# urbste/MultiCol-SLAM

Measured on AMD Instinct MI355X. Metric: Mfeatures/s extract+match, 3-cam 754x480 multi-frame, higher is better.
Workload: dtype u8+i32 (images, Hamming) / f64 (omni model)

## Files before the change

### include/mcs_c.h

```cpp
#ifndef MCS_C_H
#define MCS_C_H
#include <stdint.h>
#include <stddef.h>
#ifdef __cplusplus
extern "C" {
#endif

#define MCS_OK 0
#define MCS_ERR_INVALID (-1)
#define MCS_ERR_HIP (-2)
#define MCS_ERR_CAPACITY (-3)
#define MCS_ERR_UNSUPPORTED (-4)

#define MCS_ABI_VERSION 10

#define MCS_MAX_POLY 16
#define MCS_MAX_LEVELS 16

typedef struct mcs_ctx mcs_ctx;
typedef struct mcs_extractor mcs_extractor;

typedef struct { float x, y, size, angle, response; int32_t octave, class_id; } mcs_keypoint;

typedef struct {
// ... 43 lines not shown
int mcs_extractor_patch_ties(mcs_extractor*, int back, int* listed, int* recomputed);
int mcs_describe_fast_bound(const mcs_ocam* cam, int desc_size, double* bound);
int mcs_selftest_describe_fast(mcs_ctx*, const mcs_ocam* cam, uint64_t seed, int n, double* max_abs_diff);
int mcs_describe_fast_table(const mcs_ocam* cam, double* table, int* rows, int* row_len, int* e0, int* bins_per_octave, double* info6);
int mcs_describe_fast_table_packed(const mcs_ocam* cam, void* packed, int* row_bytes, double* f32_term);

int mcs_extract_batch_strided(mcs_extractor*, int nimg, const uint8_t* images, size_t image_pitch, int image_stride, const uint8_t* masks,
                              size_t mask_pitch, int mask_stride, const mcs_ocam* cams, int32_t* nkp, mcs_keypoint* keypoints, uint8_t* desc,
                              uint8_t* descmask, double* rays, size_t out_image_pitch_rows, int out_row_stride);

int mcs_extractor_status(mcs_extractor*);

int mcs_extractor_tap_level(mcs_extractor*, int img, int level, int blurred, uint8_t* out );
int mcs_extractor_tap_candidates(mcs_extractor*, int img, int level, uint32_t* out , int cap, int* n);
int mcs_extractor_tap_selected(mcs_extractor*, int img, int level, uint32_t* out, int cap, int* n);

typedef struct {
	const uint8_t* desc; const uint8_t* mask; const uint8_t* valid; const int32_t* group; int32_t n; int32_t stride;
	int32_t block_rows; int64_t block_pitch_rows;
} mcs_desc_set;
int mcs_match_topk(mcs_ctx*, const mcs_desc_set* q, const mcs_desc_set* t, int dim, int K, int count_thresh, mcs_mem_kind kind,
                   int32_t* out_dist, int32_t* out_idx, int32_t* out_count_le);

int mcs_match_topk_batched(mcs_ctx*, int nsets, const mcs_desc_set* q, size_t q_set_pitch_rows, const mcs_desc_set* t,
                           size_t t_set_pitch_rows, int dim, int K, int count_thresh, mcs_mem_kind kind, int32_t* out_dist,
                           int32_t* out_idx, int32_t* out_count_le);

int mcs_search_kf_kf(mcs_ctx*, int nsets, const mcs_desc_set* kf1, size_t pitch1_rows, const mcs_desc_set* kf2, size_t pitch2_rows, int dim,
                     double nnratio, int K, mcs_mem_kind kind, int32_t* match12, int32_t* nmatches, int32_t* fallbacks );
int mcs_search_kf_f(mcs_ctx*, int nsets, const mcs_desc_set* kf, size_t pitchKF_rows, const mcs_desc_set* frame, size_t pitchF_rows, int dim,
// ... 156 lines not shown
```

### multicol-slam_amd/__init__.py

```python
import ctypes as C

import numpy as np

from . import _capi
from ._capi import (KP_DTYPE, MASKS_RESIDENT, MEM_DEVICE, MEM_HOST, DescSet, ExtractorParams, McsError, Ocam, check, lib, make_ocam, np_ptr)

__all__ = ["Context", "Extractor", "McsError", "KP_DTYPE", "make_ocam", "ExtractorParams", "MEM_HOST", "MEM_DEVICE"]


class Context:

    def __init__(self, device=0, stream=None):
        self.h = C.c_void_p()
        check(lib().mcs_ctx_create(device, C.c_void_p(stream) if stream else None, C.byref(self.h)))
        self.device = device

    def close(self):
        if getattr(self, "h", None):
            lib().mcs_ctx_destroy(self.h)
            self.h = None

    def __del__(self):
        try:
            self.close()
# ... 185 lines not shown
        check(lib().mcs_extractor_tap_level(self.h, img, level, int(blurred), np_ptr(out)))
        return out

    def _tap(self, fn, img, level):
        buf = np.zeros(1 << 17, np.uint32)
        n = C.c_int32()
        check(fn(self.h, img, level, np_ptr(buf), len(buf), C.byref(n)))
        rec = buf[:n.value]
        return (rec & 0xFFF).astype(np.int32), ((rec >> 12) & 0xFFF).astype(np.int32), (rec >> 24).astype(np.int32)

    def tap_candidates(self, img, level):
        return self._tap(lib().mcs_extractor_tap_candidates, img, level)

    def tap_selected(self, img, level):
        return self._tap(lib().mcs_extractor_tap_selected, img, level)
```

### multicol-slam_amd/_capi.py

```python
import ctypes as C
import os

import numpy as np

_HERE = os.path.dirname(os.path.abspath(__file__))
LIB_PATH = os.environ.get("MCS_HIP_LIB", os.path.join(_HERE, "libmcs_hip.so"))

MCS_OK, MCS_ERR_INVALID, MCS_ERR_HIP, MCS_ERR_CAPACITY, MCS_ERR_UNSUPPORTED = 0, -1, -2, -3, -4
MEM_HOST, MEM_DEVICE = 0, 1
MASKS_RESIDENT = C.c_void_p(1)
MAX_POLY = 16


class McsError(RuntimeError):
    def __init__(self, code, msg):
        super().__init__("libmcs_hip error %d: %s" % (code, msg))
        self.code = code


class KeyPoint(C.Structure):
    _fields_ = [("x", C.c_float), ("y", C.c_float), ("size", C.c_float), ("angle", C.c_float), ("response", C.c_float),
                ("octave", C.c_int32), ("class_id", C.c_int32)]


# ... 23 lines not shown
    o = Ocam()
    o.c, o.d, o.e, o.u0, o.v0 = cam["c"], cam["d"], cam["e"], cam["u0"], cam["v0"]
    for i, v in enumerate(cam["p"]):
        o.p[i] = v
    o.p_deg = len(cam["p"])
    for i, v in enumerate(cam["invP"]):
        o.invP[i] = v
    o.invP_deg = len(cam["invP"])
    o.width, o.height = cam["width"], cam["height"]
    return o


EXPORTS = [
    "mcs_last_error", "mcs_abi_version", "mcs_device_count", "mcs_ctx_create", "mcs_ctx_destroy", "mcs_ctx_synchronize", "mcs_extractor_create",
    "mcs_extractor_destroy", "mcs_extractor_set_masks", "mcs_extractor_kp_capacity", "mcs_extractor_levels", "mcs_extract_batch", "mcs_extractor_status",
    "mcs_extractor_tap_level", "mcs_extractor_tap_candidates", "mcs_extractor_tap_selected", "mcs_match_topk",
    "mcs_match_topk_batched", "mcs_descriptor_distance", "mcs_descriptor_distance_masked", "mcs_ctx_enable_timing",
    "mcs_ctx_kernel_ms", "mcs_ctx_join", "mcs_ctx_set_async_search", "mcs_ctx_search_fence", "mcs_search_kf_kf", "mcs_search_kf_f", "mcs_search_triangulation", "mcs_search_kf_f_sweep",
    "mcs_search_triangulation_sweep", "mcs_search_kf_kf_ring", "mcs_rows_valid", "mcs_extractor_set_describe", "mcs_extractor_describe_stats", "mcs_extractor_tie_stats", "mcs_extractor_set_tie_band", "mcs_extractor_fix_ties", "mcs_extractor_tie_counts", "mcs_extractor_set_tie_capture", "mcs_extractor_patch_ties", "mcs_describe_fast_bound",
    "mcs_selftest_describe_fast", "mcs_describe_fast_table", "mcs_describe_fast_table_packed", "mcs_extract_batch_strided", "mcs_rig_pack_headers", "mcs_rig_rows_valid",
    "mcs_search_by_projection", "mcs_window_match", "mcs_window_best", "mcs_rotation_consistency", "mcs_world_to_cam", "mcs_distinctive_descriptors", "mcs_selftest_shared_reciprocal", "mcs_vocabulary_create", "mcs_vocabulary_destroy", "mcs_bow_transform", "mcs_copy_narrow", "mcs_ctx_result_stream", "mcs_ctx_stream_conflicts", "mcs_ctx_transfer_stream", "mcs_host_alloc", "mcs_host_free",
    "mcs_vocabulary_set_words", "mcs_bow_vector", "mcs_kfdb_create", "mcs_kfdb_destroy", "mcs_kfdb_clear", "mcs_kfdb_size", "mcs_kfdb_add", "mcs_kfdb_erase",
    "mcs_kfdb_set_covisibility", "mcs_kfdb_detect_relocalisation", "mcs_kfdb_detect_loop", "mcs_kfdb_score",
    "mcs_sim3_create", "mcs_sim3_destroy", "mcs_sim3_set_ransac_parameters", "mcs_sim3_iterate", "mcs_sim3_best", "mcs_sim3_info",
    "mcs_sim3_hypotheses", "mcs_sim3_draw",
    "mcs_triangulate_matches", "mcs_create_new_map_points",
    "mcs_frustum", "mcs_search_local_points",
]

WINDOW_RATIO, WINDOW_BEST, WINDOW_INITIALIZE = 1, 2, 3

# ... 85 lines not shown
    L.mcs_extractor_fix_ties.argtypes = [vp, C.POINTER(C.c_int)]
    L.mcs_extractor_set_tie_capture.argtypes = [vp, C.c_int, C.c_int]
    L.mcs_extractor_patch_ties.argtypes = [vp, C.c_int, C.POINTER(C.c_int), C.POINTER(C.c_int)]
    L.mcs_extractor_tie_counts.argtypes = [vp, C.POINTER(C.c_uint64), C.POINTER(C.c_uint64), C.POINTER(C.c_double)]
    L.mcs_describe_fast_bound.argtypes = [C.POINTER(Ocam), C.c_int, C.POINTER(C.c_double)]
    L.mcs_selftest_describe_fast.argtypes = [vp, C.POINTER(Ocam), C.c_uint64, C.c_int, C.POINTER(C.c_double)]
    L.mcs_describe_fast_table.argtypes = [C.POINTER(Ocam), vp, C.POINTER(C.c_int), C.POINTER(C.c_int), C.POINTER(C.c_int), C.POINTER(C.c_int), vp]
    L.mcs_describe_fast_table_packed.argtypes = [C.POINTER(Ocam), vp, C.POINTER(C.c_int), C.POINTER(C.c_double)]
    L.mcs_extract_batch.argtypes = [vp, C.c_int, vp, C.c_size_t, C.c_int, vp, C.c_size_t, C.c_int, vp, C.c_int, vp, vp, vp, vp, vp]
    L.mcs_extract_batch_strided.argtypes = [vp, C.c_int, vp, C.c_size_t, C.c_int, vp, C.c_size_t, C.c_int, vp, vp, vp, vp, vp, vp, C.c_size_t, C.c_int]
    L.mcs_rig_pack_headers.argtypes = [vp, vp, C.c_int, C.c_int, vp, C.c_int]
    L.mcs_rig_rows_valid.argtypes = [vp, vp, C.c_int, C.c_int, C.c_int, vp, vp]
    L.mcs_extractor_tap_level.argtypes = [vp, C.c_int, C.c_int, C.c_int, vp]
    L.mcs_extractor_tap_candidates.argtypes = [vp, C.c_int, C.c_int, vp, C.c_int, i32p]
    L.mcs_extractor_tap_selected.argtypes = [vp, C.c_int, C.c_int, vp, C.c_int, i32p]
    L.mcs_match_topk.argtypes = [vp, C.POINTER(DescSet), C.POINTER(DescSet), C.c_int, C.c_int, C.c_int, C.c_int, vp, vp, vp]
    L.mcs_match_topk_batched.argtypes = [vp, C.c_int, C.POINTER(DescSet), C.c_size_t, C.POINTER(DescSet), C.c_size_t, C.c_int,
                                         C.c_int, C.c_int, C.c_int, vp, vp, vp]
    srch = [vp, C.c_int, C.POINTER(DescSet), C.c_size_t, C.POINTER(DescSet), C.c_size_t, C.c_int, C.c_double, C.c_int, C.c_int, vp, vp, vp]
    L.mcs_search_kf_kf.argtypes = srch
    L.mcs_search_kf_f.argtypes = srch
    L.mcs_search_triangulation.argtypes = [vp, C.c_int, C.POINTER(DescSet), C.c_size_t, C.POINTER(DescSet), C.c_size_t, vp, vp, vp, C.c_int,
                                           C.c_int, C.c_int, C.c_int, vp, vp, vp]
    L.mcs_search_kf_kf_ring.argtypes = [vp, C.c_int, C.c_int, C.c_int, C.POINTER(DescSet), C.c_size_t, C.c_int, C.c_double, C.c_int, C.c_int, vp, vp, vp]
    L.mcs_search_kf_f_sweep.argtypes = [vp, C.c_int, C.POINTER(DescSet), C.c_size_t, C.c_int, C.POINTER(DescSet), C.c_size_t, C.c_int, C.c_double, C.c_int,
                                        C.c_int, vp, vp, vp]
    L.mcs_search_triangulation_sweep.argtypes = [vp, C.c_int, C.POINTER(DescSet), C.c_size_t, C.POINTER(DescSet), C.c_size_t, vp, vp, vp, C.c_size_t,
                                                 C.c_int, C.c_int, C.c_int, C.c_int, vp, vp, vp]
    L.mcs_rows_valid.argtypes = [vp, vp, C.c_int, C.c_int, vp]
    L.mcs_search_by_projection.argtypes = [vp, C.POINTER(ProjectionSet), C.POINTER(FrameView), C.c_double, C.c_double, C.c_int, C.c_int, vp, vp]
# ... 54 lines not shown
```

### multicol-slam_amd/csrc/mcs_capi.hip

```cpp
#include "mcs_common.h"

#include <algorithm>
#include <cmath>
#include <cstdio>
#include <cstdlib>
#include <cstring>
#include <map>
#include <string>
#include <vector>

namespace mcs {
bool upload_describe_tables(const signed char* pattern);
void launch_single_distance(const uint8_t* a, const uint8_t* b, const uint8_t* ma, const uint8_t* mb, int dim, int* out, hipStream_t s);
void describe_host(int mode, int descSize, const signed char* pattern, const OcamDev* cam, int undistort, int level, float levelScale, int row, int col, float angle,
                   const HostLevel& L, uint8_t* desc, uint8_t* mask);
void launch_tie_capture(const ExtractBuffers& b, const PyrDesc& hd, int nimg, int maxTies, uint8_t* devOut, hipStream_t s);
void launch_selftest_fast_model(const OcamDev* cam, const double* tab, unsigned long long seed, int n, int width, int height, unsigned long long* maxDiff, hipStream_t s);
static const signed char kPattern[2048] = {
#include "learned_pattern_64_orb.inc"
};
}

using namespace mcs;

// ... 192 lines not shown
	int* d_fbCount = nullptr; uint32_t *d_fbList = nullptr, *d_preList = nullptr; unsigned long long* d_fbStats = nullptr; unsigned long long* d_tieMin = nullptr; void* d_aux = nullptr;
	int describeMode = 0; double guardEps = kDefaultGuardEps;
	uint32_t* d_tieList = nullptr; double tieBand = 0.0; unsigned long long tieFixed = 0;
	struct TieSlot { uint8_t* host = nullptr; uint8_t* dev = nullptr; hipEvent_t ev = nullptr; ExtractBuffers b{}; int nimg = 0; std::vector<OcamDev> cams; long long seq = -1; bool patched = false; };
	std::vector<TieSlot> tieRing; int tieMax = 0; long long batchSeq = 0; hipStream_t patchStream = nullptr; uint8_t* h_patchRows = nullptr;
	unsigned long long tieWindowMisses = 0;
	TieSlot hostTie;
	struct CamFast { OcamDev key; GTabInfo info; std::vector<double> tab; };
	std::vector<CamFast> camCache;
	double* d_gTab = nullptr;
	DevBuf inImg, inMask;
	int* d_nkp = nullptr; mcs_keypoint* d_kps = nullptr; uint8_t *d_odesc = nullptr, *d_omask = nullptr; double* d_rays = nullptr;
	ExtractBuffers last{};
	int lastN = 0;
	uint8_t* d_resMask = nullptr; int resMaskN = 0;
	int* h_status = nullptr;
	struct Graph { ExtractBuffers key; int nimg; hipGraphExec_t exec; };
	std::vector<Graph> graphs;
	long graphHits = 0, graphMisses = 0;
};

extern "C" {

const char* mcs_last_error(void) { return mcs_err().c_str(); }
int mcs_abi_version(void) { return MCS_ABI_VERSION; }

int mcs_device_count(int* n) {
	if (!n) return fail(MCS_ERR_INVALID, "null");
	HIPCHK(hipGetDeviceCount(n));
	return MCS_OK;
// ... 281 lines not shown
	for (int v = -kHalfPatch; v <= kHalfPatch; ++v)
		for (int u = -umax[std::abs(v)]; u <= umax[std::abs(v)]; ++u) { disc.push_back((signed char)u); disc.push_back((signed char)v); }
	if (disc.size() != 845 * 2) { delete e; return fail(MCS_ERR_INVALID, "internal: disc size"); }
	for (int v = 0; v <= kHalfPatch; ++v) hd.umax[v] = umax[v];
	if (!upload_describe_tables(kPattern)) { delete e; return fail(MCS_ERR_HIP, "pattern tables: upload failed (or the distinct-point rounds of mcs_describe.hip do not fit this pattern)"); }

	hd.chainFits = 0; hd.chainRegOff = 0;
	if (getenv("MCS_PYR_CHAIN") && !taps.empty()) {
		std::vector<int> table;
		if (pyramid_chain_table(hd, taps.data(), &table)) {
			hd.chainFits = 1; hd.chainRegOff = (int)taps.size();
			taps.resize(taps.size() + (table.size() * sizeof(int) + sizeof(ResizeTap) - 1) / sizeof(ResizeTap));
			memcpy(taps.data() + hd.chainRegOff, table.data(), table.size() * sizeof(int));
		}
	}
	const size_t B = max_batch;
#define ALLOC(ptr, bytes) do { hipError_t _e = hipMalloc((void**)&(ptr), (bytes)); if (_e != hipSuccess) { mcs_extractor_destroy(e); return fail(MCS_ERR_HIP, std::string("hipMalloc ") + #ptr + ": " + hipGetErrorString(_e)); } } while (0)
	ALLOC(e->d_desc, sizeof(PyrDesc));
	ALLOC(e->d_cells, sizeof(CellInfo) * e->cells.size());
	ALLOC(e->d_taps, sizeof(ResizeTap) * std::max<size_t>(taps.size(), 1));
	ALLOC(e->d_maskMap, sizeof(short) * maps.size());
	ALLOC(e->d_pyr, B * hd.pyrBytes);
	ALLOC(e->d_blur, B * hd.pyrBytes);
	ALLOC(e->d_slots, B * hd.slotsPerImage * sizeof(uint32_t));
	ALLOC(e->d_dense, B * hd.densePerImage * sizeof(uint32_t));
	ALLOC(e->d_knode, B * hd.densePerImage * sizeof(unsigned short));
	ALLOC(e->d_sel, B * hd.selPerImage * sizeof(uint32_t));
	ALLOC(e->d_selAngle, B * hd.selPerImage * sizeof(float));
	ALLOC(e->d_cellCount, B * hd.cellsPerImage * sizeof(int));
	ALLOC(e->d_denseCount, B * nl * sizeof(int));
	ALLOC(e->d_selCount, B * nl * sizeof(int));
	ALLOC(e->d_status, sizeof(int));
	ALLOC(e->d_cams, B * sizeof(OcamDev));
	const size_t slotsPerImage = (size_t)(hd.kpCap + kSlotAlign - 1) / kSlotAlign * kSlotAlign;
	ALLOC(e->d_fbCount, 3 * sizeof(int));
	if (hipHostMalloc((void**)&e->h_status, 2 * sizeof(int), hipHostMallocDefault) != hipSuccess) { (void)hipGetLastError(); e->h_status = nullptr; }
	ALLOC(e->d_tieList, B * slotsPerImage * sizeof(uint32_t));
	ALLOC(e->d_fbList, B * slotsPerImage * sizeof(uint32_t));
	ALLOC(e->d_preList, B * slotsPerImage * sizeof(uint32_t));
	ALLOC(e->d_fbStats, 2 * sizeof(unsigned long long));
	ALLOC(e->d_tieMin, sizeof(unsigned long long));
	ALLOC(e->d_aux, B * slotsPerImage * describe_aux_bytes());
	ALLOC(e->d_gTab, B * (size_t)kGDevDoubles * sizeof(double));
	ALLOC(e->d_nkp, B * sizeof(int));
	ALLOC(e->d_kps, B * hd.kpCap * sizeof(mcs_keypoint));
	ALLOC(e->d_odesc, B * hd.kpCap * (size_t)hd.descSize);
	ALLOC(e->d_omask, B * hd.kpCap * (size_t)hd.descSize);
	ALLOC(e->d_rays, B * hd.kpCap * 3 * sizeof(double));
#undef ALLOC
	HIPCHK(hipMemcpy(e->d_desc, &hd, sizeof(PyrDesc), hipMemcpyHostToDevice));
	HIPCHK(hipMemcpy(e->d_cells, e->cells.data(), sizeof(CellInfo) * e->cells.size(), hipMemcpyHostToDevice));
	if (!taps.empty()) HIPCHK(hipMemcpy(e->d_taps, taps.data(), sizeof(ResizeTap) * taps.size(), hipMemcpyHostToDevice));
	HIPCHK(hipMemcpy(e->d_maskMap, maps.data(), sizeof(short) * maps.size(), hipMemcpyHostToDevice));
	HIPCHK(hipMemset(e->d_status, 0, sizeof(int)));
	HIPCHK(hipMemset(e->d_fbCount, 0, 3 * sizeof(int)));
	HIPCHK(hipMemset(e->d_fbStats, 0, 2 * sizeof(unsigned long long)));
	{ const unsigned long long inf = 0x7FF0000000000000ull; HIPCHK(hipMemcpy(e->d_tieMin, &inf, sizeof(inf), hipMemcpyHostToDevice)); }
	if (hipHostMalloc((void**)&e->hostTie.host, sizeof(TieCaptureHeader) + (size_t)kHostTieSlots * sizeof(TieCaptureEntry), hipHostMallocDefault) == hipSuccess) {
		memset(e->hostTie.host, 0, sizeof(TieCaptureHeader));
		e->hostTie.dev = (uint8_t*)device_view(e->hostTie.host);
	} else { (void)hipGetLastError(); e->hostTie.host = nullptr; }
	if (getenv("MCS_DESCRIBE_EXACT")) e->describeMode = 1;
	HIPCHK(hipMemset(e->d_pyr, 0, B * hd.pyrBytes));
	HIPCHK(hipMemset(e->d_blur, 0, B * hd.pyrBytes));
	ctx->extractors.push_back(e);
	*out = e;
// ... 5 lines not shown
	e->tieRing.clear(); e->tieMax = 0;
	if (e->h_patchRows) { (void)hipHostFree(e->h_patchRows); e->h_patchRows = nullptr; }
	if (e->patchStream) { (void)hipStreamSynchronize(e->patchStream); (void)hipStreamDestroy(e->patchStream); e->patchStream = nullptr; }
}

int mcs_extractor_destroy(mcs_extractor* e) {
	if (!e) return MCS_OK;
	(void)hipSetDevice(e->ctx->device);
	(void)hipStreamSynchronize(e->ctx->stream);
	{
		std::vector<mcs_extractor*>& v = e->ctx->extractors;
		v.erase(std::remove(v.begin(), v.end(), e), v.end());
	}
	void* ptrs[] = {e->d_desc, e->d_cells, e->d_taps, e->d_maskMap, e->d_pyr, e->d_blur, e->d_slots, e->d_dense, e->d_knode,
	                e->d_sel, e->d_cellCount, e->d_denseCount, e->d_selCount, e->d_status, e->d_cams, e->d_nkp, e->d_kps, e->d_odesc,
	                e->d_omask, e->d_rays, e->d_fbCount, e->d_fbList, e->d_preList, e->d_fbStats, e->d_tieMin, e->d_aux, e->d_gTab, e->d_selAngle, e->d_tieList};
	for (void* p : ptrs) (void)hipFree(p);
	for (mcs_extractor::Graph& g : e->graphs) (void)hipGraphExecDestroy(g.exec);
	(void)hipFree(e->d_resMask);
	if (e->h_status) (void)hipHostFree(e->h_status);
	free_tie_capture(e);
	if (e->hostTie.host) (void)hipHostFree(e->hostTie.host);
	delete e;
	return MCS_OK;
}

int mcs_extractor_kp_capacity(const mcs_extractor* e, int* cap) {
	if (!e || !cap) return fail(MCS_ERR_INVALID, "null");
	*cap = e->hd.kpCap;
	return MCS_OK;
}
// ... 177 lines not shown
		HIPCHK(hipMemcpyAsync(e->inImg.p, images, imgSpan, hipMemcpyHostToDevice, s));
		b.img0 = e->inImg.p; b.img0Pitch = image_pitch; b.img0Stride = image_stride;
		if (resMask) { b.mask0 = masks; b.mask0Pitch = mask_pitch; b.mask0Stride = mask_stride; }
		else if (masks) {
			const size_t maskSpan = (size_t)(nimg - 1) * mask_pitch + (size_t)(hd.height - 1) * mask_stride + hd.width;
			HIPCHK(e->inMask.reserve(maskSpan));
			HIPCHK(hipMemcpyAsync(e->inMask.p, masks, maskSpan, hipMemcpyHostToDevice, s));
			b.mask0 = e->inMask.p; b.mask0Pitch = mask_pitch; b.mask0Stride = mask_stride;
		}
		b.nkp = e->d_nkp; b.kps = e->d_kps; b.out_desc = e->d_odesc; b.out_mask = e->d_omask; b.rays = rays ? e->d_rays : nullptr;
	} else {
		b.img0 = images; b.img0Pitch = image_pitch; b.img0Stride = image_stride;
		b.mask0 = masks; b.mask0Pitch = mask_pitch; b.mask0Stride = mask_stride;
		b.nkp = nkp; b.kps = keypoints; b.out_desc = desc; b.out_mask = descmask; b.rays = rays;
	}
	if (cams) {
		std::vector<OcamDev> hc(nimg);
		std::vector<int> which(nimg), uniq;
		for (int i = 0; i < nimg; ++i) {
			const mcs_ocam& m = cams[i];
			OcamDev& o = hc[i];
			if (int r = ocam_to_dev(m, &o)) return r;
			int w = -1;
			for (size_t k = 0; k < e->camCache.size() && w < 0; ++k) if (memcmp(&e->camCache[k].key, &o, sizeof(o)) == 0) w = (int)k;
			if (w < 0) {
				mcs_extractor::CamFast cf;
				cf.key = o; cf.tab.assign(kGTabDoubles, 0.0);
				cf.info = build_g_table(m, cf.tab.data());
				if (!std::isfinite(cf.info.tailU)) cf.tab.assign(kGTabDoubles, 0.0);
				e->camCache.push_back(std::move(cf));
// ... 10 lines not shown
			HIPCHK(hipStreamSynchronize(s));
			HIPCHK(hipMemcpy(e->d_cams, hc.data(), sizeof(OcamDev) * hc.size(), hipMemcpyHostToDevice));
			std::vector<double> tabs(uniq.size() * (size_t)kGDevDoubles);
			for (size_t i = 0; i < uniq.size(); ++i) pack_g_table(e->camCache[uniq[i]].tab.data(), reinterpret_cast<uint8_t*>(&tabs[i * kGDevDoubles]));
			HIPCHK(hipMemcpy(e->d_gTab, tabs.data(), tabs.size() * sizeof(double), hipMemcpyHostToDevice));
			e->h_cams = hc;
		}
		if (e->camCache.size() > 64) e->camCache.clear();
		b.cams = e->d_cams;
	}
	const bool forked = c->overlap() && (long long)nimg * hd.width * hd.height >= 4000000ll;
	bool replayed = false;
	if (forked) {
		HIPCHK(hipEventRecord(c->evFork, s));
		HIPCHK(hipStreamWaitEvent(c->side, c->evFork, 0));
		if (hd.chainFits) {
			launch_pyramid(b, hd, nimg, c->side);
			HIPCHK(hipEventRecord(c->evPyr, c->side));
			launch_blur(b, hd, nimg, c->side);
			HIPCHK(hipEventRecord(c->evBlur, c->side));
			launch_fast(b, hd, nimg, s, 0, 1);
			HIPCHK(hipStreamWaitEvent(s, c->evPyr, 0));
			launch_fast(b, hd, nimg, s, 1, hd.nlevels);
		} else {
			launch_pyramid(b, hd, nimg, c->side, 1, hd.nlevels);
			HIPCHK(hipEventRecord(c->evPyr, c->side));
			launch_blur(b, hd, nimg, c->side);
			HIPCHK(hipEventRecord(c->evBlur, c->side));
			HIPCHK(hipStreamWaitEvent(s, c->evPyr, 0));
			launch_fast(b, hd, nimg, s, 0, hd.nlevels);
		}
		launch_octree(b, hd, nimg, s);
		HIPCHK(hipStreamWaitEvent(s, c->evBlur, 0));
	} else if (!c->timing && use_graphs() && !(e->graphMisses > 8 && e->graphMisses > e->graphHits)) {
		hipGraphExec_t exec = nullptr;
		for (mcs_extractor::Graph& g : e->graphs)
			if (g.nimg == nimg && memcmp(&g.key, &b, sizeof(b)) == 0) exec = g.exec;
		if (exec) ++e->graphHits; else ++e->graphMisses;
		if (!exec) {
			hipGraph_t graph = nullptr;
			hipError_t ge = hipStreamBeginCapture(s, hipStreamCaptureModeRelaxed);
			if (ge == hipSuccess) {
				launch_pyramid(b, hd, nimg, s);
				launch_fast(b, hd, nimg, s);
				launch_octree(b, hd, nimg, s);
				launch_blur(b, hd, nimg, s);
				launch_describe(b, hd, nimg, s);
				const hipError_t le = hipGetLastError();
				ge = hipStreamEndCapture(s, &graph);
				if (ge == hipSuccess && le != hipSuccess) ge = le;
				if (ge == hipSuccess) ge = hipGraphInstantiate(&exec, graph, nullptr, nullptr, 0);
				if (graph) (void)hipGraphDestroy(graph);
			}
			if (ge != hipSuccess) {
				(void)hipGetLastError();
				exec = nullptr;
				e->graphMisses = 1000000;
			} else {
				if (e->graphs.size() >= 4) { (void)hipStreamSynchronize(s); (void)hipGraphExecDestroy(e->graphs.front().exec); e->graphs.erase(e->graphs.begin()); }
				e->graphs.push_back(mcs_extractor::Graph{b, nimg, exec});
			}
		}
		if (!exec) {
			launch_pyramid(b, hd, nimg, s);
			launch_fast(b, hd, nimg, s);
			launch_octree(b, hd, nimg, s);
			launch_blur(b, hd, nimg, s);
			launch_describe(b, hd, nimg, s);
			replayed = true;
		} else {
		HIPCHK(hipGraphLaunch(exec, s));
		replayed = true;
		}
	} else {
		c->tic("pyramid"); launch_pyramid(b, hd, nimg, s); c->toc("pyramid");
		c->tic("fast"); launch_fast(b, hd, nimg, s); c->toc("fast");
		c->tic("octree"); launch_octree(b, hd, nimg, s); c->toc("octree");
		c->tic("blur"); launch_blur(b, hd, nimg, s); c->toc("blur");
	}
	if (forked) { b.sideStream = c->side; b.evDescFork = c->evDescFork; b.evDescJoin = c->evDescJoin; }
	if (!replayed) {
		ExtractBuffers bd = b;
		if (c->timing) {
			Timer& t = c->timers["describe_fast"];
			if (!t.a) { (void)hipEventCreate(&t.a); (void)hipEventCreate(&t.b); }
			bd.evFastA = t.a; bd.evFastB = t.b; t.used = true;
		}
		c->tic("describe"); launch_describe(bd, hd, nimg, s); c->toc("describe");
	}
	HIPCHK(hipGetLastError());
	e->last = b; e->lastN = nimg;
// ... 38 lines not shown
	return MCS_OK;
}

int mcs_extractor_set_masks(mcs_extractor* e, int nimg, const uint8_t* masks, size_t mask_pitch, int mask_stride, mcs_mem_kind kind) {
	if (!e || !masks || nimg < 1 || nimg > e->maxBatch) return fail(MCS_ERR_INVALID, "bad argument");
	const PyrDesc& hd = e->hd;
	if (mask_stride < hd.width) return fail(MCS_ERR_INVALID, "stride smaller than the image width");
	HIPCHK(hipSetDevice(e->ctx->device));
	HIPCHK(hipStreamSynchronize(e->ctx->stream));
	const size_t plane = (size_t)hd.width * hd.height;
	if (nimg > e->resMaskN) { (void)hipFree(e->d_resMask); e->d_resMask = nullptr; e->resMaskN = 0; HIPCHK(hipMalloc((void**)&e->d_resMask, plane * nimg)); }
	for (int i = 0; i < nimg; ++i)
		HIPCHK(hipMemcpy2D(e->d_resMask + (size_t)i * plane, hd.width, masks + (size_t)i * mask_pitch, mask_stride, hd.width, hd.height,
		                   kind == MCS_MEM_HOST ? hipMemcpyHostToDevice : hipMemcpyDeviceToDevice));
	e->resMaskN = nimg;
	return MCS_OK;
}

int mcs_extract_batch(mcs_extractor* e, int nimg, const uint8_t* images, size_t image_pitch, int image_stride, const uint8_t* masks,
                      size_t mask_pitch, int mask_stride, const mcs_ocam* cams, mcs_mem_kind kind, int32_t* nkp, mcs_keypoint* keypoints,
                      uint8_t* desc, uint8_t* descmask, double* rays) {
	return extract_impl(e, nimg, images, image_pitch, image_stride, masks, mask_pitch, mask_stride, cams, kind, nkp, keypoints, desc, descmask, rays, 0, 0);
}

int mcs_extract_batch_strided(mcs_extractor* e, int nimg, const uint8_t* images, size_t image_pitch, int image_stride, const uint8_t* masks,
                              size_t mask_pitch, int mask_stride, const mcs_ocam* cams, int32_t* nkp, mcs_keypoint* keypoints, uint8_t* desc,
                              uint8_t* descmask, double* rays, size_t out_image_pitch_rows, int out_row_stride) {
	return extract_impl(e, nimg, images, image_pitch, image_stride, masks, mask_pitch, mask_stride, cams, MCS_MEM_DEVICE, nkp, keypoints, desc, descmask, rays,
	                    out_image_pitch_rows, out_row_stride);
}
// ... 192 lines not shown
                    int cap, int* n) {
	HIPCHK(hipStreamSynchronize(e->ctx->stream));
	int cnt = 0;
	HIPCHK(hipMemcpy(&cnt, counts + (size_t)img * e->hd.nlevels + level, sizeof(int), hipMemcpyDeviceToHost));
	*n = cnt;
	const int m = std::min(cnt, cap);
	if (m > 0) HIPCHK(hipMemcpy(out, base + (size_t)img * perImage + lvBase, (size_t)m * sizeof(uint32_t), hipMemcpyDeviceToHost));
	return MCS_OK;
}

int mcs_extractor_tap_candidates(mcs_extractor* e, int img, int level, uint32_t* out, int cap, int* n) {
	if (!e || !out || !n || img < 0 || img >= e->lastN || level < 0 || level >= e->hd.nlevels) return fail(MCS_ERR_INVALID, "bad tap");
	return tap_list(e, img, level, e->d_dense, e->d_denseCount, e->hd.densePerImage, e->hd.lv[level].denseBase, out, cap, n);
}

int mcs_extractor_tap_selected(mcs_extractor* e, int img, int level, uint32_t* out, int cap, int* n) {
	if (!e || !out || !n || img < 0 || img >= e->lastN || level < 0 || level >= e->hd.nlevels) return fail(MCS_ERR_INVALID, "bad tap");
	return tap_list(e, img, level, e->d_sel, e->d_selCount, e->hd.selPerImage, e->hd.lv[level].selBase, out, cap, n);
}

}
```

### multicol-slam_amd/csrc/mcs_common.h

```cpp
#pragma once
#include <hip/hip_runtime.h>
#include <vector>
#include <stdint.h>
#include "../../include/mcs_c.h"

namespace mcs {

constexpr int kEdge = 25;
constexpr int kHalfPatch = 16;
constexpr int kPatchSize = 32;
constexpr int kMinBorder = kEdge - 3;
constexpr int kCellW = 30;
constexpr int kMaxRoots = 32;
constexpr int kMaxNodes = 2048;
constexpr int kNumXCD = 8;

struct LevelInfo {
	int w, h, stride;
	int off;
	int nCols, nRows, wCell, hCell;
	int cellBase;
	int capc;
	int slotBase;
	int denseBase, denseCap;
// ... 17 lines not shown
	int kpCap;
	int fastThreshold;
	int fastRing;
	int agast;
	int descSize, npoints;
	int umax[kHalfPatch + 1];
	int chainFits;
	int chainRegOff;
	int mode;
	int undistort;
	LevelInfo lv[MCS_MAX_LEVELS];
};

struct CellInfo { short level; short x0, y0; short cw, ch; short pad; int slot; int rowM, grpM; };

struct ResizeTap { short ofs; short a0; short a1; short pad; };

struct OcamDev {
	double c, d, e, u0, v0, invAffine;
	double p[MCS_MAX_POLY];
	double invP[MCS_MAX_POLY];
	int p_deg, invP_deg;
	int fastOk;
	int tabIdx;
};

#ifndef MCS_G_M
#define MCS_G_M 5
#define MCS_G_DEG 6
#endif
// ... 21 lines not shown
		d8 = reinterpret_cast<double*>(base);
		lvl = reinterpret_cast<int*>(d8 + (size_t)8 * nslots); rc = lvl + nslots; poff = reinterpret_cast<unsigned*>(rc + nslots);
	}
};
struct ExtractBuffers {
	const PyrDesc* desc;
	const CellInfo* cells;
	const ResizeTap* taps;
	const short* maskMap;
	const uint8_t* img0; size_t img0Pitch; int img0Stride;
	const uint8_t* mask0; size_t mask0Pitch; int mask0Stride;
	uint8_t* pyr;
	uint8_t* blur;
	uint32_t* slots;
	int* cellCount;
	uint32_t* dense;
	unsigned short* knode;
	int* denseCount;
	uint32_t* sel;
	int* selCount;
	float* selAngle;
	const OcamDev* cams;
	int* status;
	const double* gTab;
	void* aux;
	int* fbCount; uint32_t* fbList;
	int* preCount; uint32_t* preList;
	unsigned long long* fbStats;
	unsigned long long* tieMin;
	int* tieCount; uint32_t* tieList;
// ... 10 lines not shown
struct HostLevel { const uint8_t* blur; const uint8_t* raw; int w, h; const uint8_t* patch = nullptr; int prow = 0, pcol = 0, pdim = 0; bool* miss = nullptr; };
constexpr int kTiePatchR = 40;
constexpr int kTiePatchDim = 2 * kTiePatchR + 1;
struct TieCaptureHeader { int count; int status; int pad[14]; };
struct TieCaptureEntry { uint32_t gw; int level; uint32_t rec; float angle; uint8_t patch[kTiePatchDim * kTiePatchDim + 15]; };

__host__ __device__ inline const uint8_t* level_ptr(const ExtractBuffers& b, const PyrDesc& d, int img, int level, int* stride) {
	if (level == 0) { *stride = b.img0Stride; return b.img0 + (size_t)img * b.img0Pitch; }
	*stride = d.lv[level].stride;
	return b.pyr + (size_t)img * d.pyrBytes + d.lv[level].off;
}

void launch_pyramid(const ExtractBuffers& b, const PyrDesc& hd, int nimg, hipStream_t s, int level0 = 1, int level1 = MCS_MAX_LEVELS);
bool pyramid_chain_table(const PyrDesc& d, const ResizeTap* taps, std::vector<int>* table);
void launch_fast(const ExtractBuffers& b, const PyrDesc& hd, int nimg, hipStream_t s, int level0 = 0, int level1 = MCS_MAX_LEVELS);
void launch_octree(const ExtractBuffers& b, const PyrDesc& hd, int nimg, hipStream_t s, int level0 = 0, int level1 = MCS_MAX_LEVELS);
void launch_blur(const ExtractBuffers& b, const PyrDesc& hd, int nimg, hipStream_t s);
void launch_describe(const ExtractBuffers& b, const PyrDesc& hd, int nimg, hipStream_t s);
size_t describe_aux_bytes();

struct RowMap {
	size_t base; int blk; size_t bpitch;
	__device__ __forceinline__ size_t operator()(int i) const {
		if (blk == 0) return base + (size_t)i;
		const int b = i / blk;
		return base + (size_t)b * bpitch + (size_t)(i - b * blk);
	}
};

struct MatchArgs {
// ... 125 lines not shown
```

### multicol-slam_amd/csrc/mcs_fast.hip

```cpp
#include "mcs_common.h"

#include <algorithm>
#include <cstdio>
#include <cstdlib>

namespace mcs {

#ifndef MCS_FAST_BS
#define MCS_FAST_BS 128
#endif
template <int CW> struct FastGeom {
	static constexpr int kTileX = 4;
	static constexpr int kTilePitch = (CW + kTileX + 3 + 4 + 3) / 4 * 4, kTileRows = CW + 6;
	static constexpr int kScPitch = (CW + 2 + 3) / 4 * 4, kScRows = CW + 2;
};

template <int P, int kTilePitch> struct Ring;
template <int kTilePitch> struct Ring<12, kTilePitch> {
	static __device__ __forceinline__ void diffs(const uint8_t* c, int (&d)[12]) {
		const int v = c[0];
		d[0] = v - c[2 * kTilePitch]; d[1] = v - c[2 * kTilePitch + 1]; d[2] = v - c[kTilePitch + 2]; d[3] = v - c[2];
		d[4] = v - c[-kTilePitch + 2]; d[5] = v - c[-2 * kTilePitch + 1]; d[6] = v - c[-2 * kTilePitch]; d[7] = v - c[-2 * kTilePitch - 1];
		d[8] = v - c[-kTilePitch - 2]; d[9] = v - c[-2]; d[10] = v - c[kTilePitch - 2]; d[11] = v - c[2 * kTilePitch - 1];
	}
// ... 208 lines not shown
	constexpr bool kOrdered = P == 16 && AG < 0;
	__shared__ int waveTot[kFastBS / 64];
	int listRun = 0;

	const int logical = (blockIdx.x % kNumXCD) * perXcd + blockIdx.x / kNumXCD;
	if (logical >= nblocks) return;
	const PyrDesc& d = *b.desc;
	const int img = (int)__umulhi((unsigned)logical, ncellsM);
	const int ci = cell0 + (logical - img * ncells);
	const CellInfo cell = b.cells[ci];
	const LevelInfo& L = d.lv[cell.level];
	const int tid = threadIdx.x;
	const int cw = cell.cw, ch = cell.ch;
	int* countOut = b.cellCount + (size_t)img * d.cellsPerImage + ci;
	if (cw <= 0 || ch <= 0) { if (tid == 0) *countOut = 0; return; }

	int stride;
	const uint8_t* src = level_ptr(b, d, img, cell.level, &stride);
	src += (size_t)(cell.y0 - 3) * stride + (cell.x0 - Geo::kTileX);
	const int th = ch + 6;
	const bool stage16 = cell.x0 - Geo::kTileX + kTilePitch <= L.w;
	if (stage16) {
		constexpr int kChunks = (kTilePitch + 15) / 16, kLast = kTilePitch - 16;
		static_assert((kChunks & (kChunks - 1)) == 0 || kChunks == 3 || kChunks == 5 || kChunks == 6, "chunks per row");
		const int nch = kChunks * th;
		for (int c = tid; c < nch; c += kFastBS) {
			const unsigned ty = kChunks == 4 ? (unsigned)c >> 2 : kChunks == 8 ? (unsigned)c >> 3 : (unsigned)c / (unsigned)kChunks;
			const unsigned k = (unsigned)c - ty * (unsigned)kChunks;
			const unsigned xo = min(16u * k, (unsigned)kLast);
			uint4 v;
// ... 263 lines not shown
	}
	__syncthreads();
	for (int i = tid; i < ns; i += kFastBS) {
		const int p = surv[i];
		const uint32_t w = keepBits[p >> 5];
		if ((w >> (p & 31)) & 1u) {
			const int py = p >> 6, px = p & 63;
			const uint32_t below = (p & 32) ? __popc(keepBits[2 * py]) + __popc(w & ((1u << (p & 31)) - 1u)) : __popc(w & ((1u << (p & 31)) - 1u));
			const int s0 = sc[(py + 1) * kScPitch + px + 1];
			slots[rowOff[py] + (int)below] = (uint32_t)(cell.x0 + px - kMinBorder) | ((uint32_t)(cell.y0 + py - kMinBorder) << 12) | ((uint32_t)s0 << 24);
		}
	}
	if (tid == 0) *countOut = runBase;
}

void launch_fast(const ExtractBuffers& b, const PyrDesc& hd, int nimg, hipStream_t s, int level0, int level1) {
	if (level1 > hd.nlevels) level1 = hd.nlevels;
	if (level0 >= level1) return;
	const int cell0 = hd.lv[level0].cellBase;
	const int cellEnd = level1 < hd.nlevels ? hd.lv[level1].cellBase : hd.cellsPerImage;
	const int ncells = cellEnd - cell0;
	const int nblocks = nimg * ncells;
	if (nblocks <= 0) return;
	const int perXcd = (nblocks + kNumXCD - 1) / kNumXCD;
	int cellMax = 0;
	for (int l = level0; l < level1; ++l) cellMax = std::max(cellMax, std::max(hd.lv[l].wCell, hd.lv[l].hCell));
	const dim3 grid(perXcd * kNumXCD);
	if ((unsigned long long)nblocks * (unsigned long long)ncells >= (1ull << 32)) { fprintf(stderr, "mcs: FAST launch too large (%d blocks)\n", nblocks); abort(); }
	const unsigned ncellsM = (unsigned)(((1ull << 32) + (unsigned long long)ncells - 1ull) / (unsigned long long)ncells);
#define MCS_FAST_LAUNCH(P)                                                                                                                      \
// ... 27 lines not shown
```

Baseline: 143.1.

## Skip FAST cells whose mapped mask region is fully empty

Precomputes for each FAST cell the bounding rectangle of its level-0 mask coordinates. A new kernel reduces the mask into an 8x8-block occupancy bitmap in shared memory and marks each cell live or dead. The FAST kernel then exits early for dead cells. For resident masks the live flags are computed once when the masks are set, and for per-call masks an extra kernel launches every call. This removes FAST work in masked-out fisheye regions, at the cost of an additional launch and mask read per call when masks are not resident.

```diff
diff --git a/include/mcs_c.h b/include/mcs_c.h
--- a/include/mcs_c.h
+++ b/include/mcs_c.h
@@ -81,6 +81,7 @@
 int mcs_extractor_tap_level(mcs_extractor*, int img, int level, int blurred, uint8_t* out );
 int mcs_extractor_tap_candidates(mcs_extractor*, int img, int level, uint32_t* out , int cap, int* n);
 int mcs_extractor_tap_selected(mcs_extractor*, int img, int level, uint32_t* out, int cap, int* n);
+int mcs_extractor_tap_cells(mcs_extractor*, int img, int32_t (*out)[6], int cap, int* n);
 
 typedef struct {
 	const uint8_t* desc; const uint8_t* mask; const uint8_t* valid; const int32_t* group; int32_t n; int32_t stride;
diff --git a/multicol-slam_amd/__init__.py b/multicol-slam_amd/__init__.py
--- a/multicol-slam_amd/__init__.py
+++ b/multicol-slam_amd/__init__.py
@@ -223,3 +223,10 @@
 
     def tap_selected(self, img, level):
         return self._tap(lib().mcs_extractor_tap_selected, img, level)
+
+    def tap_cells(self, img):
+        buf = np.zeros((1 << 16, 6), np.int32)
+        n = C.c_int32()
+        check(lib().mcs_extractor_tap_cells(self.h, img, np_ptr(buf), len(buf), C.byref(n)))
+        assert n.value <= len(buf)
+        return buf[:n.value].copy()
diff --git a/multicol-slam_amd/_capi.py b/multicol-slam_amd/_capi.py
--- a/multicol-slam_amd/_capi.py
+++ b/multicol-slam_amd/_capi.py
@@ -61,7 +61,7 @@
 EXPORTS = [
     "mcs_last_error", "mcs_abi_version", "mcs_device_count", "mcs_ctx_create", "mcs_ctx_destroy", "mcs_ctx_synchronize", "mcs_extractor_create",
     "mcs_extractor_destroy", "mcs_extractor_set_masks", "mcs_extractor_kp_capacity", "mcs_extractor_levels", "mcs_extract_batch", "mcs_extractor_status",
-    "mcs_extractor_tap_level", "mcs_extractor_tap_candidates", "mcs_extractor_tap_selected", "mcs_match_topk",
+    "mcs_extractor_tap_level", "mcs_extractor_tap_candidates", "mcs_extractor_tap_selected", "mcs_extractor_tap_cells", "mcs_match_topk",
     "mcs_match_topk_batched", "mcs_descriptor_distance", "mcs_descriptor_distance_masked", "mcs_ctx_enable_timing",
     "mcs_ctx_kernel_ms", "mcs_ctx_join", "mcs_ctx_set_async_search", "mcs_ctx_search_fence", "mcs_search_kf_kf", "mcs_search_kf_f", "mcs_search_triangulation", "mcs_search_kf_f_sweep",
     "mcs_search_triangulation_sweep", "mcs_search_kf_kf_ring", "mcs_rows_valid", "mcs_extractor_set_describe", "mcs_extractor_describe_stats", "mcs_extractor_tie_stats", "mcs_extractor_set_tie_band", "mcs_extractor_fix_ties", "mcs_extractor_tie_counts", "mcs_extractor_set_tie_capture", "mcs_extractor_patch_ties", "mcs_describe_fast_bound",
@@ -177,6 +177,8 @@
     L.mcs_extractor_tap_level.argtypes = [vp, C.c_int, C.c_int, C.c_int, vp]
     L.mcs_extractor_tap_candidates.argtypes = [vp, C.c_int, C.c_int, vp, C.c_int, i32p]
     L.mcs_extractor_tap_selected.argtypes = [vp, C.c_int, C.c_int, vp, C.c_int, i32p]
+    if hasattr(L, "mcs_extractor_tap_cells"):
+        L.mcs_extractor_tap_cells.argtypes = [vp, C.c_int, vp, C.c_int, i32p]
     L.mcs_match_topk.argtypes = [vp, C.POINTER(DescSet), C.POINTER(DescSet), C.c_int, C.c_int, C.c_int, C.c_int, vp, vp, vp]
     L.mcs_match_topk_batched.argtypes = [vp, C.c_int, C.POINTER(DescSet), C.c_size_t, C.POINTER(DescSet), C.c_size_t, C.c_int,
                                          C.c_int, C.c_int, C.c_int, vp, vp, vp]
diff --git a/multicol-slam_amd/csrc/mcs_capi.hip b/multicol-slam_amd/csrc/mcs_capi.hip
--- a/multicol-slam_amd/csrc/mcs_capi.hip
+++ b/multicol-slam_amd/csrc/mcs_capi.hip
@@ -230,6 +230,7 @@
 	ExtractBuffers last{};
 	int lastN = 0;
 	uint8_t* d_resMask = nullptr; int resMaskN = 0;
+	CellRect* d_cellRects = nullptr; uint8_t *d_cellLive = nullptr, *d_resLive = nullptr; bool cellSkip = false;
 	int* h_status = nullptr;
 	struct Graph { ExtractBuffers key; int nimg; hipGraphExec_t exec; };
 	std::vector<Graph> graphs;
@@ -541,6 +542,22 @@
 			memcpy(taps.data() + hd.chainRegOff, table.data(), table.size() * sizeof(int));
 		}
 	}
+	std::vector<CellRect> rects(e->cells.size());
+	for (size_t i = 0; i < e->cells.size(); ++i) {
+		const CellInfo& c = e->cells[i];
+		const LevelInfo& L = hd.lv[c.level];
+		CellRect r{1, 1, 0, 0};
+		if (c.cw > 0 && c.ch > 0) {
+			const auto mx = std::minmax_element(maps.begin() + L.mapX + c.x0, maps.begin() + L.mapX + c.x0 + c.cw);
+			const auto my = std::minmax_element(maps.begin() + L.mapY + c.y0, maps.begin() + L.mapY + c.y0 + c.ch);
+			r = CellRect{*mx.first, *my.first, *mx.second, *my.second};
+		}
+		rects[i] = r;
+	}
+	{
+		const char* sw = getenv("MCS_FAST_CELL_SKIP");
+		e->cellSkip = !(sw && atoi(sw) == 0) && cell_live_fits(hd) && !rects.empty();
+	}
 	const size_t B = max_batch;
 #define ALLOC(ptr, bytes) do { hipError_t _e = hipMalloc((void**)&(ptr), (bytes)); if (_e != hipSuccess) { mcs_extractor_destroy(e); return fail(MCS_ERR_HIP, std::string("hipMalloc ") + #ptr + ": " + hipGetErrorString(_e)); } } while (0)
 	ALLOC(e->d_desc, sizeof(PyrDesc));
@@ -555,6 +572,11 @@
 	ALLOC(e->d_sel, B * hd.selPerImage * sizeof(uint32_t));
 	ALLOC(e->d_selAngle, B * hd.selPerImage * sizeof(float));
 	ALLOC(e->d_cellCount, B * hd.cellsPerImage * sizeof(int));
+	if (e->cellSkip) {
+		ALLOC(e->d_cellRects, sizeof(CellRect) * rects.size());
+		ALLOC(e->d_cellLive, B * hd.cellsPerImage);
+		ALLOC(e->d_resLive, B * hd.cellsPerImage);
+	}
 	ALLOC(e->d_denseCount, B * nl * sizeof(int));
 	ALLOC(e->d_selCount, B * nl * sizeof(int));
 	ALLOC(e->d_status, sizeof(int));
@@ -577,6 +599,7 @@
 #undef ALLOC
 	HIPCHK(hipMemcpy(e->d_desc, &hd, sizeof(PyrDesc), hipMemcpyHostToDevice));
 	HIPCHK(hipMemcpy(e->d_cells, e->cells.data(), sizeof(CellInfo) * e->cells.size(), hipMemcpyHostToDevice));
+	if (e->cellSkip) HIPCHK(hipMemcpy(e->d_cellRects, rects.data(), sizeof(CellRect) * rects.size(), hipMemcpyHostToDevice));
 	if (!taps.empty()) HIPCHK(hipMemcpy(e->d_taps, taps.data(), sizeof(ResizeTap) * taps.size(), hipMemcpyHostToDevice));
 	HIPCHK(hipMemcpy(e->d_maskMap, maps.data(), sizeof(short) * maps.size(), hipMemcpyHostToDevice));
 	HIPCHK(hipMemset(e->d_status, 0, sizeof(int)));
@@ -612,7 +635,8 @@
 	}
 	void* ptrs[] = {e->d_desc, e->d_cells, e->d_taps, e->d_maskMap, e->d_pyr, e->d_blur, e->d_slots, e->d_dense, e->d_knode,
 	                e->d_sel, e->d_cellCount, e->d_denseCount, e->d_selCount, e->d_status, e->d_cams, e->d_nkp, e->d_kps, e->d_odesc,
-	                e->d_omask, e->d_rays, e->d_fbCount, e->d_fbList, e->d_preList, e->d_fbStats, e->d_tieMin, e->d_aux, e->d_gTab, e->d_selAngle, e->d_tieList};
+	                e->d_omask, e->d_rays, e->d_fbCount, e->d_fbList, e->d_preList, e->d_fbStats, e->d_tieMin, e->d_aux, e->d_gTab, e->d_selAngle, e->d_tieList,
+	                e->d_cellRects, e->d_cellLive, e->d_resLive};
 	for (void* p : ptrs) (void)hipFree(p);
 	for (mcs_extractor::Graph& g : e->graphs) (void)hipGraphExecDestroy(g.exec);
 	(void)hipFree(e->d_resMask);
@@ -820,6 +844,9 @@
 		b.mask0 = masks; b.mask0Pitch = mask_pitch; b.mask0Stride = mask_stride;
 		b.nkp = nkp; b.kps = keypoints; b.out_desc = desc; b.out_mask = descmask; b.rays = rays;
 	}
+	const bool liveCall = e->cellSkip && b.mask0 && !resMask;
+	if (e->cellSkip && b.mask0) b.cellLive = resMask ? e->d_resLive : e->d_cellLive;
+	auto cell_live = [&](hipStream_t st) { if (liveCall) launch_cell_live(b, hd, e->d_cellRects, e->d_cellLive, nimg, st); };
 	if (cams) {
 		std::vector<OcamDev> hc(nimg);
 		std::vector<int> which(nimg), uniq;
@@ -860,6 +887,7 @@
 	if (forked) {
 		HIPCHK(hipEventRecord(c->evFork, s));
 		HIPCHK(hipStreamWaitEvent(c->side, c->evFork, 0));
+		cell_live(s);
 		if (hd.chainFits) {
 			launch_pyramid(b, hd, nimg, c->side);
 			HIPCHK(hipEventRecord(c->evPyr, c->side));
@@ -888,6 +916,7 @@
 			hipError_t ge = hipStreamBeginCapture(s, hipStreamCaptureModeRelaxed);
 			if (ge == hipSuccess) {
 				launch_pyramid(b, hd, nimg, s);
+				cell_live(s);
 				launch_fast(b, hd, nimg, s);
 				launch_octree(b, hd, nimg, s);
 				launch_blur(b, hd, nimg, s);
@@ -909,6 +938,7 @@
 		}
 		if (!exec) {
 			launch_pyramid(b, hd, nimg, s);
+			cell_live(s);
 			launch_fast(b, hd, nimg, s);
 			launch_octree(b, hd, nimg, s);
 			launch_blur(b, hd, nimg, s);
@@ -920,7 +950,7 @@
 		}
 	} else {
 		c->tic("pyramid"); launch_pyramid(b, hd, nimg, s); c->toc("pyramid");
-		c->tic("fast"); launch_fast(b, hd, nimg, s); c->toc("fast");
+		c->tic("fast"); cell_live(s); launch_fast(b, hd, nimg, s); c->toc("fast");
 		c->tic("octree"); launch_octree(b, hd, nimg, s); c->toc("octree");
 		c->tic("blur"); launch_blur(b, hd, nimg, s); c->toc("blur");
 	}
@@ -989,6 +1019,14 @@
 		HIPCHK(hipMemcpy2D(e->d_resMask + (size_t)i * plane, hd.width, masks + (size_t)i * mask_pitch, mask_stride, hd.width, hd.height,
 		                   kind == MCS_MEM_HOST ? hipMemcpyHostToDevice : hipMemcpyDeviceToDevice));
 	e->resMaskN = nimg;
+	if (e->cellSkip) {
+		ExtractBuffers b{};
+		b.mask0 = e->d_resMask; b.mask0Pitch = plane; b.mask0Stride = hd.width;
+		HIPCHK(hipStreamSynchronize(nullptr));
+		launch_cell_live(b, hd, e->d_cellRects, e->d_resLive, nimg, e->ctx->stream);
+		HIPCHK(hipGetLastError());
+		HIPCHK(hipStreamSynchronize(e->ctx->stream));
+	}
 	return MCS_OK;
 }
 
@@ -1211,6 +1249,20 @@
 	return tap_list(e, img, level, e->d_dense, e->d_denseCount, e->hd.densePerImage, e->hd.lv[level].denseBase, out, cap, n);
 }
 
+int mcs_extractor_tap_cells(mcs_extractor* e, int img, int32_t (*out)[6], int cap, int* n) {
+	if (!e || !out || !n || img < 0 || img >= e->lastN || cap < 0) return fail(MCS_ERR_INVALID, "bad tap");
+	HIPCHK(hipStreamSynchronize(e->ctx->stream));
+	const int nc = (int)e->cells.size();
+	std::vector<uint8_t> live(nc, 1);
+	if (e->last.cellLive && nc > 0) HIPCHK(hipMemcpy(live.data(), e->last.cellLive + (size_t)img * nc, nc, hipMemcpyDeviceToHost));
+	*n = nc;
+	for (int i = 0; i < std::min(nc, cap); ++i) {
+		const CellInfo& c = e->cells[i];
+		out[i][0] = c.level; out[i][1] = c.x0; out[i][2] = c.y0; out[i][3] = c.cw; out[i][4] = c.ch; out[i][5] = live[i];
+	}
+	return MCS_OK;
+}
+
 int mcs_extractor_tap_selected(mcs_extractor* e, int img, int level, uint32_t* out, int cap, int* n) {
 	if (!e || !out || !n || img < 0 || img >= e->lastN || level < 0 || level >= e->hd.nlevels) return fail(MCS_ERR_INVALID, "bad tap");
 	return tap_list(e, img, level, e->d_sel, e->d_selCount, e->hd.selPerImage, e->hd.lv[level].selBase, out, cap, n);
diff --git a/multicol-slam_amd/csrc/mcs_common.h b/multicol-slam_amd/csrc/mcs_common.h
--- a/multicol-slam_amd/csrc/mcs_common.h
+++ b/multicol-slam_amd/csrc/mcs_common.h
@@ -55,6 +55,8 @@
 
 struct CellInfo { short level; short x0, y0; short cw, ch; short pad; int slot; int rowM, grpM; };
 
+struct CellRect { short x0, y0, x1, y1; };
+
 struct ResizeTap { short ofs; short a0; short a1; short pad; };
 
 struct OcamDev {
@@ -106,6 +108,7 @@
 	uint8_t* blur;
 	uint32_t* slots;
 	int* cellCount;
+	const uint8_t* cellLive;
 	uint32_t* dense;
 	unsigned short* knode;
 	int* denseCount;
@@ -146,6 +149,8 @@
 void launch_pyramid(const ExtractBuffers& b, const PyrDesc& hd, int nimg, hipStream_t s, int level0 = 1, int level1 = MCS_MAX_LEVELS);
 bool pyramid_chain_table(const PyrDesc& d, const ResizeTap* taps, std::vector<int>* table);
 void launch_fast(const ExtractBuffers& b, const PyrDesc& hd, int nimg, hipStream_t s, int level0 = 0, int level1 = MCS_MAX_LEVELS);
+bool cell_live_fits(const PyrDesc& hd);
+void launch_cell_live(const ExtractBuffers& b, const PyrDesc& hd, const CellRect* rects, uint8_t* live, int nimg, hipStream_t s);
 void launch_octree(const ExtractBuffers& b, const PyrDesc& hd, int nimg, hipStream_t s, int level0 = 0, int level1 = MCS_MAX_LEVELS);
 void launch_blur(const ExtractBuffers& b, const PyrDesc& hd, int nimg, hipStream_t s);
 void launch_describe(const ExtractBuffers& b, const PyrDesc& hd, int nimg, hipStream_t s);
diff --git a/multicol-slam_amd/csrc/mcs_fast.hip b/multicol-slam_amd/csrc/mcs_fast.hip
--- a/multicol-slam_amd/csrc/mcs_fast.hip
+++ b/multicol-slam_amd/csrc/mcs_fast.hip
@@ -246,6 +246,7 @@
 	const int cw = cell.cw, ch = cell.ch;
 	int* countOut = b.cellCount + (size_t)img * d.cellsPerImage + ci;
 	if (cw <= 0 || ch <= 0) { if (tid == 0) *countOut = 0; return; }
+	if (b.cellLive && b.cellLive[(size_t)img * d.cellsPerImage + ci] == 0) { if (tid == 0) *countOut = 0; return; }
 
 	int stride;
 	const uint8_t* src = level_ptr(b, d, img, cell.level, &stride);
@@ -539,6 +540,77 @@
 	if (tid == 0) *countOut = runBase;
 }
 
+constexpr int kLiveBS = 1024;
+__device__ __forceinline__ void live_mark(uint32_t* grid, int gy, int pitchW, int gx) { atomicOr(&grid[gy * pitchW + (gx >> 5)], 1u << (gx & 31)); }
+__global__ __launch_bounds__(kLiveBS) void k_cell_live(const uint8_t* __restrict__ mask0, size_t maskPitch, int maskStride, int w, int h, const CellRect* __restrict__ rects,
+                                                       int ncells, uint8_t* __restrict__ live, int pitchW) {
+	extern __shared__ uint32_t liveGrid[];
+	const int img = blockIdx.x, tid = threadIdx.x;
+	const uint8_t* m = mask0 + (size_t)img * maskPitch;
+	const int GH = (h + 7) >> 3;
+	for (int i = tid; i < GH * pitchW; i += kLiveBS) liveGrid[i] = 0u;
+	__syncthreads();
+	if (w >= 16) {
+		const int chunks = (w + 15) >> 4, last = w - 16, units = GH * chunks;
+		for (int u = tid; u < units; u += kLiveBS) {
+			const int gy = u / chunks, k = u - gy * chunks;
+			const int xo = min(16 * k, last);
+			uint4 acc = uint4{0u, 0u, 0u, 0u};
+#pragma unroll
+			for (int r = 0; r < 8; ++r) {
+				const int y = min(8 * gy + r, h - 1);
+				uint4 v;
+				__builtin_memcpy(&v, m + ((size_t)y * maskStride + xo), 16);
+				acc.x |= v.x; acc.y |= v.y; acc.z |= v.z; acc.w |= v.w;
+			}
+			if ((xo & 7) == 0) {
+				if (acc.x | acc.y) live_mark(liveGrid, gy, pitchW, xo >> 3);
+				if (acc.z | acc.w) live_mark(liveGrid, gy, pitchW, (xo >> 3) + 1);
+			} else {
+				const uint32_t a[4] = {acc.x, acc.y, acc.z, acc.w};
+				uint32_t cols = 0;
+#pragma unroll
+				for (int i = 0; i < 16; ++i)
+					if ((a[i >> 2] >> (8 * (i & 3))) & 0xffu) cols |= 1u << (((xo + i) >> 3) - (xo >> 3));
+				for (int c = 0; c < 3; ++c)
+					if ((cols >> c) & 1u) live_mark(liveGrid, gy, pitchW, (xo >> 3) + c);
+			}
+		}
+	} else {
+		for (int u = tid; u < GH * w; u += kLiveBS) {
+			const int gy = u / w, x = u - gy * w;
+			uint32_t any = 0;
+			for (int r = 0; r < 8; ++r) any |= m[(size_t)min(8 * gy + r, h - 1) * maskStride + x];
+			if (any) live_mark(liveGrid, gy, pitchW, x >> 3);
+		}
+	}
+	__syncthreads();
+	for (int c = tid; c < ncells; c += kLiveBS) {
+		const CellRect r = rects[c];
+		uint32_t any = 0;
+		if (r.x0 > r.x1) any = 1u;
+		else {
+			const int gx0 = r.x0 >> 3, gx1 = r.x1 >> 3, w0 = gx0 >> 5, w1 = gx1 >> 5;
+			for (int gy = r.y0 >> 3; gy <= (r.y1 >> 3); ++gy)
+				for (int wd = w0; wd <= w1; ++wd) {
+					uint32_t sel = ~0u;
+					if (wd == w0) sel &= ~0u << (gx0 & 31);
+					if (wd == w1) sel &= ~0u >> (31 - (gx1 & 31));
+					any |= liveGrid[gy * pitchW + wd] & sel;
+				}
+		}
+		live[(size_t)img * ncells + c] = any ? 1 : 0;
+	}
+}
+
+static int live_grid_bytes(const PyrDesc& hd) { return ((hd.height + 7) / 8) * (((hd.width + 7) / 8 + 31) / 32) * (int)sizeof(uint32_t); }
+bool cell_live_fits(const PyrDesc& hd) { return live_grid_bytes(hd) <= 64 * 1024; }
+void launch_cell_live(const ExtractBuffers& b, const PyrDesc& hd, const CellRect* rects, uint8_t* live, int nimg, hipStream_t s) {
+	if (!b.mask0 || !rects || !live || nimg <= 0 || hd.cellsPerImage <= 0) return;
+	hipLaunchKernelGGL(k_cell_live, dim3(nimg), dim3(kLiveBS), live_grid_bytes(hd), s, b.mask0, b.mask0Pitch, b.mask0Stride, hd.width, hd.height, rects, hd.cellsPerImage, live,
+	                   ((hd.width + 7) / 8 + 31) / 32);
+}
+
 void launch_fast(const ExtractBuffers& b, const PyrDesc& hd, int nimg, hipStream_t s, int level0, int level1) {
 	if (level1 > hd.nlevels) level1 = hd.nlevels;
 	if (level0 >= level1) return;
```

Result: no change. 142.7 (-0.3%).
